# jeffreyhorn/network_flow_solver

Measured on AMD Instinct MI355X. Metric: pivots/sec + arcs-priced/sec (value = arcs-priced/sec; pivots_per_sec alongside) on netgen_8-style DIMACS, higher is better.
Workload: dtype int64; 1 GPU; netgen_8_08a(synthetic,x1): 256 nodes / 2048 arcs; pricing=full-scan Dantzig, step=one pivot (price + ratio test + tree/potential update), parallelism=1 GPU, sweeps=full (every arc priced every pivot)

## Files before the change

### __graft_entry__.py

```python

from __future__ import annotations

import os
import re
import subprocess
import sys
from pathlib import Path

ROOT = Path(__file__).resolve().parent
PKG = ROOT / "network_flow_solver_amd"
CSRC = PKG / "csrc"
LIB = PKG / "libmcf_hip.so"
CERT_HOST_LIB = PKG / "libmcf_certify_host.so"
REPAIR_HOST_LIB = PKG / "libmcf_repair_host.so"
FARKAS_HOST_LIB = PKG / "libmcf_farkas_host.so"
TOPOLOGY_HOST_LIB = PKG / "libmcf_topology_host.so"
RANGES_HOST_LIB = PKG / "libmcf_ranges_host.so"
FLOW_RANGES_HOST_LIB = PKG / "libmcf_flow_ranges_host.so"
DUAL_HOST_LIB = PKG / "libmcf_dual_host.so"
APPLY_PATHS_HOST_LIB = PKG / "libmcf_apply_paths_host.so"
SMALL_REDUCE_HOST_LIB = PKG / "libmcf_small_reduce_host.so"
SMALL_CYCLE_REGS_HOST_LIB = PKG / "libmcf_small_cycle_regs_host.so"
FORK_HOST_LIB = PKG / "libmcf_fork_host.so"

if str(ROOT) not in sys.path:
    sys.path.insert(0, str(ROOT))


def _hipcc() -> str:
    for cand in (os.environ.get("HIPCC"), "/opt/rocm/bin/hipcc", "hipcc"):
        if cand and (os.path.isabs(cand) and os.path.exists(cand) or not os.path.isabs(cand)):
            return cand
    return "hipcc"


def _needs_rebuild(target: Path, sources) -> bool:
    if not target.exists():
        return True
    t = target.stat().st_mtime
    return any(Path(s).stat().st_mtime > t for s in sources)


def build_hip(force: bool = False) -> Path:
    sources = [CSRC / "mcf_engine.hip", CSRC / "mcf_passes_dev.h", CSRC / "mcf_passes_host.h", CSRC / "mcf_core.h", CSRC / "mcf_host.h",
               ROOT / "include" / "mcf.h"]
    if force or _needs_rebuild(LIB, sources):
        cmd = [_hipcc(), "--offload-arch=gfx950", "-O3", "-std=c++17", "-fPIC", "-shared",
               "-o", str(LIB), str(CSRC / "mcf_engine.hip")]
        subprocess.run(cmd, check=True, cwd=str(CSRC))
    return LIB


def build_certify_host(force: bool = False) -> Path:
    src = CSRC / "mcf_certify_host.cpp"
    if force or _needs_rebuild(CERT_HOST_LIB, [src, CSRC / "mcf_core.h"]):
        subprocess.run(["g++", "-O2", "-std=c++17", "-fPIC", "-shared", "-o", str(CERT_HOST_LIB), str(src)], check=True, cwd=str(CSRC))
    return CERT_HOST_LIB


def build_repair_host(force: bool = False) -> Path:
    src = CSRC / "mcf_repair_host.cpp"
    if force or _needs_rebuild(REPAIR_HOST_LIB, [src, CSRC / "mcf_core.h", CSRC / "mcf_host.h"]):
        subprocess.run(["g++", "-O2", "-std=c++17", "-fPIC", "-shared", "-o", str(REPAIR_HOST_LIB), str(src)], check=True, cwd=str(CSRC))
    return REPAIR_HOST_LIB


def build_farkas_host(force: bool = False) -> Path:
    src = CSRC / "mcf_farkas_host.cpp"
    if force or _needs_rebuild(FARKAS_HOST_LIB, [src, CSRC / "mcf_core.h"]):
        subprocess.run(["g++", "-O2", "-std=c++17", "-fPIC", "-shared", "-o", str(FARKAS_HOST_LIB), str(src)], check=True, cwd=str(CSRC))
    return FARKAS_HOST_LIB


def build_topology_host(force: bool = False) -> Path:
    src = CSRC / "mcf_topology_host.cpp"
    if force or _needs_rebuild(TOPOLOGY_HOST_LIB, [src, CSRC / "mcf_core.h", CSRC / "mcf_host.h"]):
        subprocess.run(["g++", "-O2", "-std=c++17", "-fPIC", "-shared", "-o", str(TOPOLOGY_HOST_LIB), str(src)], check=True, cwd=str(CSRC))
    return TOPOLOGY_HOST_LIB


def build_ranges_host(force: bool = False) -> Path:
    src = CSRC / "mcf_ranges_host.cpp"
    if force or _needs_rebuild(RANGES_HOST_LIB, [src, CSRC / "mcf_core.h"]):
        subprocess.run(["g++", "-O2", "-std=c++17", "-fPIC", "-shared", "-o", str(RANGES_HOST_LIB), str(src)], check=True, cwd=str(CSRC))
    return RANGES_HOST_LIB


def build_flow_ranges_host(force: bool = False) -> Path:
    src = CSRC / "mcf_flow_ranges_host.cpp"
    if force or _needs_rebuild(FLOW_RANGES_HOST_LIB, [src, CSRC / "mcf_core.h"]):
        subprocess.run(["g++", "-O2", "-std=c++17", "-fPIC", "-shared", "-o", str(FLOW_RANGES_HOST_LIB), str(src)], check=True, cwd=str(CSRC))
    return FLOW_RANGES_HOST_LIB


def build_dual_host(force: bool = False) -> Path:
    src = CSRC / "mcf_dual_host.cpp"
    if force or _needs_rebuild(DUAL_HOST_LIB, [src, CSRC / "mcf_core.h", CSRC / "mcf_host.h", ROOT / "include" / "mcf.h"]):
        subprocess.run(["g++", "-O2", "-std=c++17", "-fPIC", "-shared", "-o", str(DUAL_HOST_LIB), str(src)], check=True, cwd=str(CSRC))
    return DUAL_HOST_LIB


def build_apply_paths_host(force: bool = False) -> Path:
    src = CSRC / "mcf_apply_paths_host.cpp"
    if force or _needs_rebuild(APPLY_PATHS_HOST_LIB, [src, CSRC / "mcf_core.h", CSRC / "mcf_host.h"]):
        subprocess.run(["g++", "-O2", "-std=c++17", "-fPIC", "-shared", "-o", str(APPLY_PATHS_HOST_LIB), str(src)], check=True, cwd=str(CSRC))
    return APPLY_PATHS_HOST_LIB


def build_small_reduce_host(force: bool = False) -> Path:
    src = CSRC / "mcf_small_reduce_host.cpp"
    if force or _needs_rebuild(SMALL_REDUCE_HOST_LIB, [src, CSRC / "mcf_core.h"]):
        subprocess.run(["g++", "-O2", "-std=c++17", "-fPIC", "-shared", "-o", str(SMALL_REDUCE_HOST_LIB), str(src)], check=True, cwd=str(CSRC))
    return SMALL_REDUCE_HOST_LIB


def build_small_cycle_regs_host(force: bool = False) -> Path:
    src = CSRC / "mcf_small_cycle_regs_host.cpp"
    if force or _needs_rebuild(SMALL_CYCLE_REGS_HOST_LIB, [src, CSRC / "mcf_core.h"]):
        subprocess.run(["g++", "-O2", "-std=c++17", "-fPIC", "-shared", "-o", str(SMALL_CYCLE_REGS_HOST_LIB), str(src)], check=True, cwd=str(CSRC))
    return SMALL_CYCLE_REGS_HOST_LIB


def build_fork_host(force: bool = False) -> Path:
    src = CSRC / "mcf_fork_host.cpp"
    if force or _needs_rebuild(FORK_HOST_LIB, [src, CSRC / "mcf_core.h"]):
        subprocess.run(["g++", "-O2", "-std=c++17", "-fPIC", "-shared", "-o", str(FORK_HOST_LIB), str(src)], check=True, cwd=str(CSRC))
    return FORK_HOST_LIB


def declared_symbols() -> list[str]:
    text = (ROOT / "include" / "mcf.h").read_text()
    text = re.sub(r"/\*.*?\*/", "", text, flags=re.S)
    names = re.findall(r"\b(mcf_[a-z0-9_]+)\s*\(", text)
    return sorted(set(n for n in names if n != "mcf_progress_cb"))


def build() -> None:
    build_hip()
    import oracle

    oracle.build()
    oracle.build_emul()
    build_certify_host()
    build_repair_host()
    build_farkas_host()
    build_topology_host()
    build_ranges_host()
    build_flow_ranges_host()
    build_dual_host()
    build_apply_paths_host()
    build_small_reduce_host()
    build_small_cycle_regs_host()
    build_fork_host()
    import ctypes

    lib = ctypes.CDLL(str(LIB))
    missing = [s for s in declared_symbols() if not hasattr(lib, s)]
    if missing:
        raise RuntimeError(f"libmcf_hip.so lacks symbols declared in include/mcf.h: {missing}")
    import network_flow_solver_amd


def smoke() -> None:
    import numpy as np

    build_hip()
    import oracle
    from network_flow_solver_amd import engine, generators

    if engine.device_count() <= 0:
        raise RuntimeError("smoke() needs a GPU: no HIP device visible")
    inst = generators.netgen_style(256, 2048, seed=7)
    ref = oracle.solve_soa(inst, "dantzig")
    for rule in (engine.RULE_DANTZIG, engine.RULE_DEVEX_BLOCK, engine.RULE_CANDIDATE_LIST):
        with engine.McfEngine(inst.n, inst.tail, inst.head, inst.cost, inst.cap, inst.supply, rule=rule,
                              device=0) as eng:
            eng.solve()
            res = eng.result()
        assert res.status == ref["status"] == "optimal", (res.status, ref["status"])
        assert res.objective == int(round(ref["objective"])), (res.objective, ref["objective"])
        bal = inst.supply.astype(np.int64).copy()
        np.subtract.at(bal, inst.tail, res.flow)
        np.add.at(bal, inst.head, res.flow)
        assert not bal.any()
        rc = inst.cost + res.potential[inst.tail] - res.potential[inst.head]
        assert (rc[(res.flow > 0) & (res.flow < inst.cap)] == 0).all()
        assert (rc[(res.flow == 0) & (inst.cap > 0)] >= 0).all() and (rc[(res.flow == inst.cap) & (inst.cap > 0)] <= 0).all()
        print(f"smoke ok: rule={rule} objective={res.objective} pivots={res.stats['pivots']} "
              f"(oracle {ref['iterations']} pivots)")


if __name__ == "__main__":
    build()
    if len(sys.argv) > 1 and sys.argv[1] == "smoke":
        smoke()
```

### network_flow_solver_amd/csrc/mcf_core.h

```cpp
#pragma once
#include <stdint.h>

#if defined(__HIPCC__)
#define MCF_HD __host__ __device__ __forceinline__
#else
#define MCF_HD inline
#endif

#define MCF_INF ((int64_t)1 << 60)

#if defined(__HIP_DEVICE_COMPILE__)
#define mcf_double_bits(x) ((int64_t)__double_as_longlong(x))
#else
static inline int64_t mcf_double_bits(double x) { int64_t k; __builtin_memcpy(&k, &x, 8); return k; }
#endif

#if defined(__HIP_DEVICE_COMPILE__)
#define MCF_TEAM_BARRIER() __syncthreads()
#define MCF_ATOMIC_MIN64(p, x) atomicMin(reinterpret_cast<long long*>(p), (long long)(x))
#define MCF_ATOMIC_MIN32(p, x) atomicMin(reinterpret_cast<int*>(p), (int)(x))
#define MCF_ATOMIC_MAX32(p, x) atomicMax(reinterpret_cast<int*>(p), (int)(x))
#define MCF_ATOMIC_ADD32(p, x) atomicAdd(reinterpret_cast<int*>(p), (int)(x))
#define MCF_ATOMIC_MAX64(p, x) atomicMax(reinterpret_cast<long long*>(p), (long long)(x))
#define MCF_ATOMIC_OR32(p, x) atomicOr(reinterpret_cast<int*>(p), (int)(x))
// ... 1107 lines not shown
        c->status = MCF_UNBOUNDED;
        c->unbounded_arc = e;
        return;
    }
    if (delta == 0) c->degenerate += 1;
    c->pivots += 1;
    c->cycle_arcs += n1 + n2 + 1;
    c->pv_e = e; c->pv_s = s; c->pv_n1 = n1; c->pv_n2 = n2; c->pv_delta = delta; c->pv_result = result;
    if (v.weight) {
        bool reset = false;
        if (result != 0) {
            if (c->swaps_since_reset >= MCF_DEVEX_RESET_SWAPS) { reset = true; c->swaps_since_reset = 0; }
            else c->swaps_since_reset += 1;
        }
        if (!reset && v.dx) {
            if (c->wlist_n >= MCF_WLIST_CAP) reset = true;
            else {
                const int32_t len = n1 + n2;
                v.weight[e] = (float)(len > 0 ? len : 1);
                v.dx->wlist[c->wlist_n] = e;
                c->wlist_n += 1;
            }
        }
        if (reset) { c->wreset = 1; c->block_index = 0; }
        c->tn_total += 1;
        if (delta == 0 || result == 0) c->tn_degenerate += 1;
        if (c->auto_tune && c->pivots - c->tn_last_adapt >= 50 && c->tn_total >= 10) {
            int32_t bg = c->block_granules;
            if (10 * c->tn_degenerate > 3 * c->tn_total) {
                const int32_t nb = bg * 3 / 2 > bg + 1 ? bg * 3 / 2 : bg + 1;
                bg = nb < c->max_granules ? nb : (bg > c->max_granules ? bg : c->max_granules);
            } else if (10 * c->tn_degenerate < c->tn_total) {
                const int32_t nb = bg * 3 / 4;
                bg = nb > 1 ? nb : 1;
            }
            if (bg != c->block_granules) {
                c->block_granules = bg;
                c->num_blocks = (MCF_GRANULES + bg - 1) / bg;
                c->block_size = v.m * bg / MCF_GRANULES;
                if (c->block_index >= c->num_blocks) c->block_index = 0;
            }
            c->tn_degenerate = 0; c->tn_total = 0; c->tn_last_adapt = c->pivots;
        }
    }
    if (result == 0) {
        c->bound_flips += 1;
        c->stage = 1;
        return;
    }

    mcf_pivot_swap(v, pp, cy, result, result == 1 ? k1 : k2, 0);
}

#define MCF_DUAL_FLOW_LIMIT ((int64_t)1 << 61)

MCF_HD int64_t mcf_dual_violation(int64_t cap, int64_t flow) {
    if (flow < 0) return -flow;
    return (cap < MCF_INF && flow > cap) ? flow - cap : 0;
}
MCF_HD int32_t mcf_dual_leave_state(int64_t flow) { return flow < 0 ? 1 : -1; }
MCF_HD bool mcf_dual_exports(bool up, int64_t flow) { return up == (flow >= 0); }
MCF_HD bool mcf_dual_candidate(int32_t state, int64_t cap, bool tail_in, bool head_in, bool exports) {
    if (state == 0 || cap == 0 || tail_in == head_in) return false;
    const bool first_in = state > 0 ? tail_in : head_in;
    return first_in == exports;
}
MCF_HD int32_t mcf_dual_closed_state(int32_t state, int64_t cap, int64_t rc) {
    return (state != 0 && cap == 0 && (int64_t)state * rc < 0) ? -state : state;
}
MCF_HD bool mcf_dual_in_subtree(int32_t pos, int32_t pos_q, int32_t size_q) { return pos >= pos_q && pos < pos_q + size_q; }

struct McfDualLeave { int64_t viol; int64_t node; int64_t maxabs; };
MCF_HD void mcf_acc_init(McfDualLeave* a) { a->viol = 0; a->node = -1; a->maxabs = 0; }
MCF_HD void mcf_dual_leave_add(McfDualLeave* a, int64_t viol, int64_t node, int64_t flow) {
    if (viol > 0 && (viol > a->viol || (viol == a->viol && (a->node < 0 || node < a->node)))) { a->viol = viol; a->node = node; }
    const int64_t mag = flow < 0 ? -flow : flow;
    if (mag > a->maxabs) a->maxabs = mag;
}
MCF_HD void mcf_acc_merge(McfDualLeave* a, const McfDualLeave& b) {
    if (b.node >= 0) mcf_dual_leave_add(a, b.viol, b.node, 0);
    if (b.maxabs > a->maxabs) a->maxabs = b.maxabs;
}
MCF_HD bool mcf_dual_too_large(const McfDualLeave& l) { return l.maxabs >= MCF_DUAL_FLOW_LIMIT || l.viol >= MCF_DUAL_FLOW_LIMIT; }
struct McfDualEnter { int64_t slack; int64_t arc; };
MCF_HD void mcf_acc_init(McfDualEnter* a) { a->slack = 0; a->arc = -1; }
MCF_HD void mcf_dual_enter_add(McfDualEnter* a, int64_t slack, int64_t packed_arc) {
    if (a->arc < 0 || slack < a->slack || (slack == a->slack && packed_arc < a->arc)) { a->slack = slack; a->arc = packed_arc; }
}
MCF_HD void mcf_acc_merge(McfDualEnter* a, const McfDualEnter& b) { if (b.arc >= 0) mcf_dual_enter_add(a, b.slack, b.arc); }

MCF_HD void mcf_pivot_begin_dual(const McfView& v, int64_t packed_arc, McfCycle* cy) {
    McfCtx* c = v.ctx;
    c->apply = 0;
    c->stage = 0;
    c->nchg = 0;
    if (c->wreset) { c->wreset = 0; c->wlist_n = 0; }
    if (c->pending_flip) {
        c->cur ^= 1;
        c->prev_lo = c->lo;
        c->prev_hi = c->hi;
        c->pending_flip = 0;
        if (c->rebuild) { c->arena ^= 1; c->rebuild = 0; }
    }
    if (packed_arc < 0) return;
    const int32_t e = (int32_t)(packed_arc & 0xffffffff);
    const McfArcW ae = v.arcw[e];
// ... 861 lines not shown
```

### network_flow_solver_amd/csrc/mcf_engine.hip

```cpp
#include <hip/hip_runtime.h>

#include <algorithm>
#include <cerrno>
#include <chrono>
#include <cstdio>
#include <cstdlib>
#include <cstring>
#include <mutex>
#include <new>
#include <string>
#include <vector>

#include "../../include/mcf.h"
#include "mcf_core.h"
#include "mcf_host.h"

namespace {

constexpr int kPriceThreads = 256;
constexpr int kPivotThreads = 1024;
constexpr int kReduceThreads = 256;
constexpr int kMidMaxNodes = 1536;
constexpr int kMidMaxArcsPerPivot = MCF_TUNER_MAX_ARCS + 1024;
constexpr int64_t kIncrementalMinArcs = (int64_t)1 << 22;
// ... 1287 lines not shown
template <int THREADS>
__device__ __forceinline__ void copy_words(void* dst, const void* src, uint32_t bytes) {
    const uint32_t n = bytes >> 2;
    const int32_t* s = static_cast<const int32_t*>(src);
    int32_t* d = static_cast<int32_t*>(dst);
    for (uint32_t i = threadIdx.x; i < n; i += THREADS) d[i] = s[i];
}

#ifdef MCF_STAMPS
#define STAMP(slot)                                                                       \
    do {                                                                                  \
        if (threadIdx.x == 0) {                                                           \
            const unsigned long long now_ = __builtin_amdgcn_s_memtime();                 \
            stamps_[slot] += now_ - last_;                                                \
            last_ = now_;                                                                 \
        }                                                                                 \
    } while (0)
#else
#define STAMP(slot) do {} while (0)
#endif
#ifdef MCF_STAMPS
#define MCF_LAST_WAVE_BEGIN() const unsigned long long lw0_ = __builtin_amdgcn_s_memtime()
#define MCF_LAST_WAVE_STAMP() do { last_wave_ += __builtin_amdgcn_s_memtime() - lw0_; } while (0)
#else
#define MCF_LAST_WAVE_BEGIN() do {} while (0)
#define MCF_LAST_WAVE_STAMP() do {} while (0)
#endif
#if defined(MCF_STAMPS) && defined(MCF_WAVE_STAMPS)
__shared__ unsigned long long mcf_wave_acc[16][6];
__shared__ unsigned long long mcf_wave_t0[16];
#define MCF_WAVE_T0() do { if ((threadIdx.x & 63) == 0) mcf_wave_t0[threadIdx.x >> 6] = __builtin_amdgcn_s_memtime(); } while (0)
#define MCF_WAVE_STAMP(slot)                                                                                                  \
    do { if ((threadIdx.x & 63) == 0) mcf_wave_acc[threadIdx.x >> 6][slot] += __builtin_amdgcn_s_memtime() - mcf_wave_t0[threadIdx.x >> 6]; } while (0)
#define MCF_WAVE_PROBE(word)                                                                                                  \
    do {                                                                                                                      \
        if (threadIdx.x < 64) {                                                                                               \
            const unsigned long long a_ = __builtin_amdgcn_s_memtime();                                                       \
            asm volatile("s_waitcnt lgkmcnt(0)" ::: "memory");                                                                \
            const unsigned long long b_ = __builtin_amdgcn_s_memtime();                                                       \
            asm volatile("s_waitcnt lgkmcnt(0)" ::: "memory");                                                                \
            const int32_t x_ = *reinterpret_cast<const volatile int32_t*>(word);                                              \
            asm volatile("s_waitcnt lgkmcnt(0)" ::"v"(x_) : "memory");                                                        \
            const unsigned long long c_ = __builtin_amdgcn_s_memtime();                                                       \
            asm volatile("s_waitcnt lgkmcnt(0)" ::: "memory");                                                                \
            if (threadIdx.x == 0) mcf_wave_acc[0][5] += (c_ - b_) - (b_ - a_);                                                \
        }                                                                                                                     \
    } while (0)
#else
#define MCF_WAVE_T0() do {} while (0)
#define MCF_WAVE_STAMP(slot) do {} while (0)
#define MCF_WAVE_PROBE(word) do {} while (0)
#endif

struct SmallCycleAcc {
    int32_t c1[16], c2[16];
};
constexpr bool small_search_join(int threads) { return threads != 256; }

template <bool LAST>
__device__ __forceinline__ void small_ratio_side(const int64_t* res, int32_t n, int64_t* d_out, int32_t* k_out) {
    const int32_t lane = (int32_t)(threadIdx.x & 63);
    int64_t d = MCF_INF;
    int32_t k = -1;
    const int64_t r0 = lane < n ? res[lane] : MCF_INF;
    bool wide = !mcf_ratio_narrow_ok(r0);
    for (int32_t i = 64 + lane; i < n; i += 64) wide |= !mcf_ratio_narrow_ok(res[i]);
    if (__ballot(wide) == 0) {
        for (int32_t base = 0; base < n; base += 64) {
            const int32_t i = base + lane;
            const uint32_t key = mcf_ratio_key32(base == 0 ? r0 : (i < n ? res[i] : MCF_INF));
            const uint32_t mn = mcf_wave_min_u32(key);
            const uint64_t mask = __ballot(i < n && key == mn);
            mcf_ratio_take<LAST>(mcf_ratio_unkey32(mn), mask, base, d, k);
        }
        *d_out = d; *k_out = k;
        return;
    }
    for (int32_t base = 0; base < n; base += 64) {
        const int32_t i = base + lane;
        const int64_t r = i < n ? res[i] : INT64_MAX;
        const int64_t mn = -mcf_wave_max64(-r);
        const uint64_t mask = __ballot(r == mn);
        mcf_ratio_take<LAST>(mn, mask, base, d, k);
    }
    *d_out = d; *k_out = k;
}

constexpr bool small_search_one_branch(int threads) { return threads == 256; }

constexpr bool small_ratio_together(int threads) { return threads == 256 || threads == 1024; }
constexpr bool small_record_once(int threads) { return threads == 256; }
typedef int small_i32x4 __attribute__((ext_vector_type(4)));

template <int THREADS>
__device__ __forceinline__ void small_cycle_parallel(const McfView& v, SmallCycleAcc& A, int64_t* scratch, McfCycle& cy) {
    constexpr bool kScalar = small_scalar_control(THREADS);
    constexpr bool kSearchJoin = small_search_join(THREADS);
    constexpr bool kSearchOneBranch = small_search_one_branch(THREADS);
    constexpr bool kRatioTogether = small_ratio_together(THREADS);
    constexpr bool kRecordOnce = small_record_once(THREADS);
    const McfCtx* c = v.ctx;
    const int32_t* pcur = c->cur ? v.posbuf[1] : v.posbuf[0];
    const int32_t du0 = cy.r0u.depth, dw0 = cy.r0w.depth;
    const int32_t pu = cy.p0u, pw = cy.p0w;
    const int32_t wave = (int32_t)threadIdx.x >> 6;
    const int32_t N = v.n_nodes;
    int64_t* const res1 = scratch;
    int64_t* const res2 = res1 + N;
    int32_t* const by_depth = reinterpret_cast<int32_t*>(res2 + N);
    int32_t n1w = 0, n2w = 0;
    const int32_t nx = kSearchJoin ? N : N - 1;
    for (int32_t x0 = 0; x0 < nx; x0 += THREADS) {
        const int32_t x = x0 + (int32_t)threadIdx.x;
        bool h1 = false, h2 = false;
        if (x < nx) {
            McfNode rec;
            if (kRecordOnce) {
                const small_i32x4 raw = *reinterpret_cast<const small_i32x4*>(&v.node[x]);
                rec.parent = raw.x; rec.pred = raw.y; rec.size = raw.z; rec.depth = raw.w;
            } else rec = v.node[x];
            const int32_t px = pcur[x];
            const bool au = (uint32_t)(pu - px) < (uint32_t)rec.size, aw = (uint32_t)(pw - px) < (uint32_t)rec.size;
            if (au && aw) { if (kSearchJoin) by_depth[rec.depth] = x; }
            else if (kSearchOneBranch) {
                if (au || aw) {
                    const McfArcW a = v.arcw[rec.pred >> 1];
                    const int32_t idx = (au ? du0 : dw0) - rec.depth;
                    (au ? v.path1 : v.path2)[idx] = x; (au ? v.rec1 : v.rec2)[idx] = rec; (au ? v.ppos1 : v.ppos2)[idx] = px;
                    const bool loses = ((rec.pred & 1) != 0) == au;
                    (au ? res1 : res2)[idx] = loses ? a.flow : (a.cap >= MCF_INF ? MCF_INF : a.cap - a.flow);
                    h1 = au; h2 = aw;
                }
            } else if (au) {
                const McfArcW a = v.arcw[rec.pred >> 1];
                const int32_t idx = du0 - rec.depth;
                v.path1[idx] = x; v.rec1[idx] = rec; v.ppos1[idx] = px;
                res1[idx] = (rec.pred & 1) ? a.flow : (a.cap >= MCF_INF ? MCF_INF : a.cap - a.flow);
                h1 = true;
            } else if (aw) {
                const McfArcW a = v.arcw[rec.pred >> 1];
                const int32_t idx = dw0 - rec.depth;
                v.path2[idx] = x; v.rec2[idx] = rec; v.ppos2[idx] = px;
                res2[idx] = (rec.pred & 1) ? (a.cap >= MCF_INF ? MCF_INF : a.cap - a.flow) : a.flow;
                h2 = true;
            }
        }
        n1w += (int32_t)__popcll(__ballot(h1));
        n2w += (int32_t)__popcll(__ballot(h2));
    }
    if ((threadIdx.x & 63) == 0) { A.c1[wave] = n1w; A.c2[wave] = n2w; }
    MCF_WAVE_STAMP(0);
    __syncthreads();
    int32_t n1 = 0, n2 = 0;
    int64_t d1, d2;
    int32_t k1, k2;
    {
        constexpr int kWaves = THREADS / 64;
        const int32_t lane = (int32_t)(threadIdx.x & 63);
        const int32_t c1 = lane < kWaves ? A.c1[lane] : 0, c2 = lane < kWaves ? A.c2[lane] : 0;
        const int32_t li = lane < N ? lane : N - 1;
        int64_t q1 = 0, q2 = 0;
        if (kRatioTogether) { q1 = res1[li]; q2 = res2[li]; }
#pragma unroll
        for (int q = 0; q < kWaves; ++q) { n1 += __builtin_amdgcn_readlane(c1, q); n2 += __builtin_amdgcn_readlane(c2, q); }
        bool both = false;
        if (kRatioTogether) {
            const int64_t r1 = lane < n1 ? q1 : MCF_INF, r2 = lane < n2 ? q2 : MCF_INF;
            const bool odd = !mcf_ratio_narrow_ok(r1) || !mcf_ratio_narrow_ok(r2);
            both = n1 <= 64 && n2 <= 64 && __ballot(odd) == 0;
            if (both) {
                const uint32_t key1 = mcf_ratio_key32(r1), key2 = mcf_ratio_key32(r2);
                uint32_t mn1, mn2;
                mcf_wave_min_u32_pair(key1, key2, mn1, mn2);
                const uint64_t mask1 = __ballot(lane < n1 && key1 == mn1), mask2 = __ballot(lane < n2 && key2 == mn2);
                d1 = MCF_INF; k1 = -1; d2 = MCF_INF; k2 = -1;
                if (n1 > 0) mcf_ratio_take<false>(mcf_ratio_unkey32(mn1), mask1, 0, d1, k1);
                if (n2 > 0) mcf_ratio_take<true>(mcf_ratio_unkey32(mn2), mask2, 0, d2, k2);
            }
        }
        if (!both) {
            small_ratio_side<false>(res1, n1, &d1, &k1);
            small_ratio_side<true>(res2, n2, &d2, &k2);
        }
    }
    cy.d1 = uni64<kScalar>(d1); cy.k1 = uni32<kScalar>(k1); cy.d2 = uni64<kScalar>(d2); cy.k2 = uni32<kScalar>(k2);
    cy.n1 = n1; cy.n2 = n2;
    MCF_WAVE_STAMP(1);
    if (kSearchJoin) {
        const int32_t jn = uni32<kScalar>(by_depth[du0 - n1]);
        const McfNode rj = uni_node<kScalar>(v.node[jn]);
        const int32_t pj = uni32<kScalar>(pcur[jn]);
        cy.u = jn; cy.w = jn; cy.ru = rj; cy.rw = rj;
        cy.pu = pj; cy.pw = pj; cy.su = pj; cy.sw = pj;
    }
}

enum { kSweepGeneric = 0, kSweepPlain = 1, kSweepDevex = 2 };

template <int MODE>
__device__ __forceinline__ void small_price_lds(const McfView& v, int32_t rule, bool devex, int32_t i, int64_t& key, int64_t& arc) {
    const int32_t st = v.state[i];
    const int32_t t = v.tail[i], h = v.head[i], o = v.orig[i];
    const int64_t cst = v.cost[i];
    float w = 1.0f;
    if (MODE == kSweepDevex || (MODE == kSweepGeneric && rule == MCF_RULE_DEVEX_BLOCK)) w = v.weight[i];
    const int64_t rc = cst + v.pi[t] - v.pi[h];
    const int64_t viol = st > 0 ? -rc : rc;
    if (st == 0 || viol <= 0) return;
    int64_t kk;
    int32_t id = o;
    if (MODE == kSweepPlain) kk = viol;
    else if (MODE == kSweepDevex) {
        kk = __double_as_longlong(((double)viol * (double)viol) / (double)w);
        id = mcf_devex_tie_id(o, st);
    } else {
        kk = mcf_dantzig_key(v, i, viol, st);
        if (rule == MCF_RULE_DEVEX_BLOCK) kk = __double_as_longlong(((double)viol * (double)viol) / (double)w);
        if (devex) id = mcf_devex_tie_id(o, st);
    }
    const int64_t pid = mcf_pack_arc(id, i);
    if (mcf_cand_better(kk, pid, key, arc)) { key = kk; arc = pid; }
}

__device__ __forceinline__ void half_wave_argmax(int64_t& key, int64_t& arc) {
    int64_t x = key;
    x = mcf_dpp_max_step<0xB1, 0xf>(x);
    x = mcf_dpp_max_step<0x4E, 0xf>(x);
    x = mcf_dpp_max_step<0x141, 0xf>(x);
    x = mcf_dpp_max_step<0x140, 0xf>(x);
    x = mcf_dpp_max_step<0x142, 0xa>(x);
    const int64_t m0 = readlane64(x, 31), m1 = readlane64(x, 63);
    const bool upper = (threadIdx.x & 32) != 0;
    const int64_t mx = upper ? m1 : m0;
    const uint64_t mask = __ballot(key == mx && key > 0);
    int64_t best[2] = {-1, -1};
#pragma unroll
    for (int hf = 0; hf < 2; ++hf) {
        uint64_t mk = hf ? (mask >> 32) << 32 : mask & 0xffffffffull;
        while (mk) {
            const int lane = __ffsll((unsigned long long)mk) - 1;
            const int64_t a = readlane64(arc, lane);
            if (best[hf] < 0 || a < best[hf]) best[hf] = a;
            mk &= mk - 1;
        }
    }
    const int64_t b = upper ? best[1] : best[0];
    key = b < 0 ? 0 : mx;
    arc = b;
}

constexpr bool small_desc_once(int threads, bool front) { return threads == 256 && !front; }
__device__ __forceinline__ uint32_t small_info(int32_t tail, int32_t head, int32_t q) { return (uint32_t)tail | ((uint32_t)head << 11) | ((uint32_t)q << 22); }
__device__ __forceinline__ McfCandX small_record(uint32_t info, int64_t viol, int32_t orig, int32_t e) {
    McfCandX x;
    x.state = (info >> 31) ? -1 : 1;
    x.rc = x.state > 0 ? -viol : viol;
    x.arc = mcf_pack_arc(orig, e);
    x.tail = (int32_t)(info & 0x7ff); x.head = (int32_t)((info >> 11) & 0x7ff); x.pad = 0;
    return x;
}
__device__ __forceinline__ void small_price_lds_narrow(const McfView& v, int32_t i, int32_t q, uint64_t& best, uint32_t& info) {
    const int32_t st = v.state[i];
    const int32_t t = v.tail[i], h = v.head[i], o = v.orig[i];
    const int32_t* pi32 = reinterpret_cast<const int32_t*>(v.pi);
    const int32_t rc = (int32_t)((uint32_t)v.cost[i] + (uint32_t)pi32[2 * t] - (uint32_t)pi32[2 * h]);
    const int32_t viol = st > 0 ? -rc : rc;
    const uint64_t p = ((uint64_t)(uint32_t)((st != 0 && viol > 0) ? viol : 0) << 32) | (uint32_t)~o;
    if (p > best) { best = p; info = small_info(t, h, q) | ((uint32_t)st & 0x80000000u); }
}
struct alignas(16) SmallWaveSlot {
    uint64_t key;
    int32_t e;
    uint32_t info;
};

#define MCF_SMALL_CTL_32(F)                                                                                                   \
    F(status) F(unbounded_arc) F(empty_blocks) F(num_blocks) F(block_granules) F(tn_total) F(tn_degenerate)                   \
    F(swaps_since_reset) F(wlist_n) F(wreset) F(minor_left) F(cur) F(pending_flip) F(prev_lo) F(prev_hi) F(apply) F(lo) F(hi) \
    F(nchg) F(stage) F(arena) F(rebuild)
#define MCF_SMALL_CTL_64(F)                                                                                                   \
    F(pivots) F(degenerate) F(bound_flips) F(arcs_priced) F(nodes_moved) F(subtree_nodes) F(cycle_arcs) F(block_size)         \
    F(block_index) F(tn_last_adapt) F(minor_pivots) F(major_sweeps)
#define MCF_SMALL_DESC_BEGIN_32(F) F(pv_e) F(pv_s) F(pv_first) F(pv_second) F(pv_t2n)
#define MCF_SMALL_DESC_BEGIN_64(F) F(pv_rc) F(pv_cap) F(pv_flow)
#define MCF_SMALL_DESC_DECIDE_32(F) F(pv_n1) F(pv_n2) F(pv_result)
#define MCF_SMALL_DESC_DECIDE_64(F) F(pv_delta)
#define MCF_SMALL_DESC_SWAP_32(F)                                                                                             \
    F(pv_k) F(pv_vin) F(pv_leave) F(pv_leave_state) F(pv_tail_in_t2) F(pv_vin_depth) F(pv_dd0) F(t2_old) F(t2_new) F(t2_size)  \
    F(nseg)
#define MCF_SMALL_DESC_SWAP_64(F) F(sigma)
template <bool SCALAR> __device__ __forceinline__ void small_ctx_uniform(McfCtx& x) {
#define MCF_F32(f) x.f = uni32<SCALAR>(x.f);
#define MCF_F64(f) x.f = uni64<SCALAR>(x.f);
    MCF_SMALL_CTL_32(MCF_F32) MCF_SMALL_CTL_64(MCF_F64)
    MCF_SMALL_DESC_BEGIN_32(MCF_F32) MCF_SMALL_DESC_BEGIN_64(MCF_F64)
    MCF_SMALL_DESC_DECIDE_32(MCF_F32) MCF_SMALL_DESC_DECIDE_64(MCF_F64)
    MCF_SMALL_DESC_SWAP_32(MCF_F32) MCF_SMALL_DESC_SWAP_64(MCF_F64)
    x.pv_t2node = uni32<SCALAR>(x.pv_t2node);
#undef MCF_F32
#undef MCF_F64
}
#define MCF_FST(f) c->f = x.f;
__device__ __forceinline__ void small_ctx_store(McfCtx* c, const McfCtx& x) {
    MCF_SMALL_CTL_32(MCF_FST) MCF_SMALL_CTL_64(MCF_FST)
// ... 200 lines not shown
    if (threadIdx.x == 0) { for (int i = 0; i < 24; ++i) mcf_stamp_acc[i] = 0; mcf_stamp_last = last_; }
#ifdef MCF_WAVE_STAMPS
    if (threadIdx.x < 16 * 6) (&mcf_wave_acc[0][0])[threadIdx.x] = 0;
#endif
#endif
    const SmallSizes sizes = small_sizes(g);
    McfView v = small_map_view<FRONT>(g, L, smem);
    small_copy_image<THREADS, true>(g, L, smem, v.weight != nullptr, sizes);
    __syncthreads();
    STAMP(0);

    McfCtx* const c = v.ctx;
    if (threadIdx.x == 0) arm_ctx(c, cap);
    __shared__ int32_t s_gran[MCF_NUM_BUCKETS][MCF_GRANULES + 1];
    const bool devex = !FRONT && rule == MCF_RULE_DEVEX_BLOCK && g.dx;
    small_load_granules<THREADS>(g, devex, s_gran);
    const bool listing = !FRONT && rule == MCF_RULE_CANDIDATE_LIST;
    __shared__ int64_t s_lk[MCF_NUM_BUCKETS], s_la[MCF_NUM_BUCKETS];
    if (listing && threadIdx.x < MCF_NUM_BUCKETS) { s_lk[threadIdx.x] = list[threadIdx.x].key; s_la[threadIdx.x] = list[threadIdx.x].arc; }
    __syncthreads();
    __shared__ int32_t s_gsum[MCF_GRANULES + 1];
    small_sum_granules(devex, s_gran, s_gsum);
    __syncthreads();
    constexpr bool kScalar = small_scalar_control(THREADS);
    const int64_t priced_all = uni32<kScalar>(s_gsum[MCF_GRANULES] - s_gsum[0]);

    constexpr int kPer = THREADS / MCF_NUM_BUCKETS;
    constexpr int kReg = small_reg_arcs(THREADS);
    static_assert(kPer == 32 || kPer % 64 == 0, "a head bucket's lanes are half a wave or whole waves");
    const int px = threadIdx.x / kPer, pl = threadIdx.x % kPer;
    const int sweep = FRONT ? (int)kSweepPlain
                            : (devex ? kSweepDevex : (rule != MCF_RULE_DEVEX_BLOCK && v.key_mode == MCF_KEY_PLAIN ? kSweepPlain : kSweepGeneric));
    int32_t r_tail[kReg], r_head[kReg], r_cost[kReg], r_orig[kReg];
    uint32_t r_info[kReg];
    int32_t r_n = 0;
    constexpr int kRegFew = small_reg_arcs_few(THREADS, FRONT);
    static_assert(kRegFew <= kReg, "the shorter unrolled sweep is a prefix of the longer");
    const bool even = FRONT && sweep == kSweepPlain && rule == MCF_RULE_DANTZIG;
    const int32_t r_step = even ? THREADS : kPer;
    const int32_t r_lo = even ? mcf_even_arc(s_gran[0][0], (int32_t)threadIdx.x, 0, THREADS) : s_gran[px][0] + pl;
    const int32_t r_hi = even ? s_gran[MCF_NUM_BUCKETS - 1][MCF_GRANULES] : s_gran[px][MCF_GRANULES];
    const bool r_few = even && uni32<kScalar>(mcf_even_reg_slots(s_gran[MCF_NUM_BUCKETS - 1][MCF_GRANULES] - s_gran[0][0], THREADS, kRegFew, kReg)) == kRegFew;
#pragma unroll
    for (int k = 0; k < kReg; ++k) {
        const int32_t i = r_lo + k * r_step;
        const bool on = sweep == kSweepPlain && i < r_hi;
        r_tail[k] = on ? v.tail[i] : 0; r_head[k] = on ? v.head[i] : 0; r_cost[k] = on ? v.cost[i] : 0; r_orig[k] = on ? v.orig[i] : 0;
        r_info[k] = small_info(r_tail[k], r_head[k], k);
        r_n += on ? 1 : 0;
    }
    const bool reg_plain = sweep == kSweepPlain;
    constexpr bool nar = FRONT;
    constexpr bool kDescOnce = small_desc_once(THREADS, FRONT);
    constexpr bool hand = FRONT;
    const int32_t* const pi32 = reinterpret_cast<const int32_t*>(v.pi);
    McfCtx cx = *c;
    small_ctx_uniform<kScalar>(cx);
    cx.max_pivots = uni64<kScalar>(cx.max_pivots); cx.minor_cap = uni32<kScalar>(cx.minor_cap); cx.auto_tune = uni32<kScalar>(cx.auto_tune);
    cx.devex_cyclic = uni32<kScalar>(cx.devex_cyclic); cx.max_granules = uni32<kScalar>(cx.max_granules);
    v.ctx = &cx;
    const int64_t adj2 = uni64<kScalar>(cx.pv_adj[2]), adj3 = uni64<kScalar>(cx.pv_adj[3]);
    int64_t* const scratch = reinterpret_cast<int64_t*>(smem + L.scratch);
    __shared__ McfCycle s_cy;
    __shared__ int s_ok;
    __shared__ SmallCycleAcc s_acc;
    __shared__ SmallWaveSlot s_slot[THREADS / 64];
    for (;;) {
        if (cx.status != MCF_RUNNING) break;
#if defined(MCF_STAMPS) && defined(MCF_WAVE_STAMPS)
        if ((cx.pivots & 15) == 0) { MCF_WAVE_PROBE(&s_acc.c1[0]); if (threadIdx.x == 64) mcf_wave_acc[1][5] += 1; }
#endif
        MCF_WAVE_T0();
        const bool minor = listing && cx.minor_left > 0;
        int32_t bg0, bg1;
        devex_block_granules(cx, devex, bg0, bg1);
        int64_t key = 0, arc = -1;
        McfCandX wx;
        wx.rc = 0; wx.arc = -1; wx.tail = 0; wx.head = 0; wx.state = 0; wx.pad = 0;
        uint64_t nbest = 0xffffffffull;
        uint32_t info = 0;
        if (!minor) {
            if (nar) {
                auto slots = [&](auto ns) {
                    constexpr int NS = decltype(ns)::value;
                    int32_t st[NS], pt[NS], ph[NS];
#pragma unroll
                    for (int k = 0; k < NS; ++k) {
                        st[k] = v.state[k < r_n ? r_lo + k * r_step : 0];
                        pt[k] = pi32[2 * r_tail[k]];
                        ph[k] = pi32[2 * r_head[k]];
                    }
#pragma unroll
                    for (int k = 0; k < NS; ++k) {
                        const int32_t rc = (int32_t)((uint32_t)r_cost[k] + (uint32_t)pt[k] - (uint32_t)ph[k]);
                        const int32_t s = k < r_n ? st[k] : 0;
                        const int32_t viol = s > 0 ? -rc : rc;
                        const uint64_t p = ((uint64_t)(uint32_t)((s != 0 && viol > 0) ? viol : 0) << 32) | (uint32_t)~r_orig[k];
                        if (p > nbest) { nbest = p; info = r_info[k] | ((uint32_t)s & 0x80000000u); }
                    }
                };
                if (r_few) slots(SmallSlots<kRegFew>{});
                else slots(SmallSlots<kReg>{});
                int32_t q = kReg;
                for (int32_t i = r_lo + kReg * r_step; i < r_hi; i += r_step, ++q) small_price_lds_narrow(v, i, q, nbest, info);
                if (nbest >> 32) { key = (int64_t)(nbest >> 32); arc = mcf_pack_arc((int32_t)~(uint32_t)nbest, r_lo + (int32_t)((info >> 22) & 0x1ff) * r_step); }
            } else if (reg_plain) {
                auto slots = [&](auto ns) {
                    constexpr int NS = decltype(ns)::value;
                    int32_t st[NS];
                    int64_t pt[NS], ph[NS];
#pragma unroll
                    for (int k = 0; k < NS; ++k) {
                        st[k] = v.state[k < r_n ? r_lo + k * r_step : 0];
                        pt[k] = v.pi[r_tail[k]];
                        ph[k] = v.pi[r_head[k]];
                    }
#pragma unroll
                    for (int k = 0; k < NS; ++k) {
                        const int64_t rc = (int64_t)r_cost[k] + pt[k] - ph[k];
                        const int32_t s = k < r_n ? st[k] : 0;
                        const int64_t viol = s > 0 ? -rc : rc;
                        const int64_t pid = mcf_pack_arc(r_orig[k], r_lo + k * r_step);
                        if (s != 0 && viol > 0 && mcf_cand_better(viol, pid, key, arc)) { key = viol; arc = pid; }
// ... 17 lines not shown
                    __shared__ int64_t s_wk[THREADS / 64], s_wa[THREADS / 64];
                    wave_argmax(key, arc);
                    if ((threadIdx.x & 63) == 0) { s_wk[threadIdx.x >> 6] = key; s_wa[threadIdx.x >> 6] = arc; }
                    __syncthreads();
                    if (threadIdx.x < MCF_NUM_BUCKETS) {
                        const int w = kWpb * threadIdx.x;
                        int64_t bk = s_wk[w], ba = s_wa[w];
                        for (int q = 1; q < kWpb; ++q)
                            if (mcf_cand_better(s_wk[w + q], s_wa[w + q], bk, ba)) { bk = s_wk[w + q]; ba = s_wa[w + q]; }
                        s_lk[threadIdx.x] = bk; s_la[threadIdx.x] = ba;
                    }
                } else {
                    half_wave_argmax(key, arc);
                    if (pl == 0) { s_lk[px] = key; s_la[px] = arc; }
                }
                __syncthreads();
            }
            const int32_t l = (int32_t)(threadIdx.x & 63);
            key = 0; arc = -1;
            if (l < MCF_NUM_BUCKETS) {
                arc = s_la[l];
                key = minor ? mcf_minor_key(v, arc) : s_lk[l];
                if (key <= 0) { key = 0; arc = -1; }
            }
            wave_argmax(key, arc);
        } else if constexpr (FRONT) {
            small_handover_publish(nbest, arc, info, s_slot);
            __syncthreads();
            small_handover_pick<THREADS>(s_slot, key, arc, wx);
        } else {
            block_argmax_all<THREADS>(key, arc);
        }
        STAMP(2);
        if (cx.pivots < cx.max_pivots)
            cx.arcs_priced += minor ? (int64_t)MCF_NUM_BUCKETS : (devex ? (int64_t)uni32<kScalar>(s_gsum[bg1] - s_gsum[bg0]) : priced_all);
        MCF_PSTAMP(12);
        McfCycle cy;
        bool go;
        if constexpr (hand) go = mcf_pivot_begin_t<true>(v, key, arc, rule, &wx, &cy);
        else go = mcf_pivot_begin_t<true>(v, key, arc, rule, nullptr, &cy);
        small_ctx_uniform<kScalar>(cx);
        MCF_PSTAMP(13);
        if (!go) {
            STAMP(3);
            __syncthreads();
            STAMP(5);
            continue;
        }
        small_cycle_ends<kScalar>(cy);
        const int32_t deep = cy.r0u.depth > cy.r0w.depth ? cy.r0u.depth : cy.r0w.depth;
        if (v.n_nodes <= kSmallCycleMaxNodes && deep > 3) {
            small_cycle_parallel<THREADS>(v, s_acc, scratch, cy);
            MCF_PSTAMP(15);
            mcf_pivot_decide(v, mcf_view_paths(v), cy);
        } else {
            if (threadIdx.x < 2) {
                const bool ok = pivot_climb_2lanes(v, &s_cy);
                if (threadIdx.x == 0) s_ok = ok ? 1 : 0;
            }
            __syncthreads();
            if (uni32<kScalar>(s_ok)) {
                cy = s_cy;
                uni_cycle<kScalar>(cy);
                mcf_pivot_decide(v, mcf_view_paths(v), cy);
            } else {
                cx.status = MCF_INTERNAL_ERROR;
            }
        }
        small_ctx_uniform<kScalar>(cx);
        if constexpr (!kDescOnce) { if (threadIdx.x == 0) small_desc_store(c, cx, adj2, adj3); }
        MCF_PSTAMP(16);
        STAMP(3);
        MCF_WAVE_STAMP(2);
        if ((int32_t)threadIdx.x >= THREADS - 64) {
            MCF_LAST_WAVE_BEGIN();
            mcf_pivot_finish_t<true>(v, mcf_view_paths(v), (int32_t)threadIdx.x - (THREADS - 64), 64);
            MCF_LAST_WAVE_STAMP();
            MCF_WAVE_STAMP(4);
        }
        STAMP(4);
        small_apply<THREADS, FRONT>(v, cx);
        MCF_WAVE_STAMP(3);
        __syncthreads();
        cx.apply = 0;
        STAMP(5);
    }
    if (threadIdx.x == 0) {
        small_ctx_store(c, cx);
        if constexpr (kDescOnce) small_desc_store_all(c, cx);
    }
    v.ctx = c;
    __syncthreads();
    __shared__ int s_any;
    small_budget_check<THREADS>(v, g, c, s_any);
    small_copy_image<THREADS, false>(g, L, smem, v.weight != nullptr, sizes);
    if (host_ctx) copy_words<THREADS>(host_ctx, smem + L.ctx, (uint32_t)sizeof(McfCtx));
    if (listing && threadIdx.x < MCF_NUM_BUCKETS) list[threadIdx.x] = McfCand{s_lk[threadIdx.x], s_la[threadIdx.x]};
#ifdef MCF_STAMPS
    STAMP(6);
    if (threadIdx.x == 0) {
        unsigned long long* out = reinterpret_cast<unsigned long long*>(g.rec1);
        for (int i = 0; i < 7; ++i) out[i] = stamps_[i];
        for (int i = 0; i < 24; ++i) g_pivot_stamps[i] += mcf_stamp_acc[i];
    }
    if (threadIdx.x == THREADS - 64) reinterpret_cast<unsigned long long*>(g.rec1)[7] = last_wave_;
#ifdef MCF_WAVE_STAMPS
    if (threadIdx.x < 16 * 6 && (int64_t)g.n_nodes * (int64_t)sizeof(McfNode) >= (8 + 16 * 6) * 8)
// ... 2080 lines not shown
```

Before: 640.7 million arcs/s.

## Use branch-free pivot decide and packed wave counts in small-graph kernel

Adds a branch-free, predicated version of mcf_pivot_decide for the 256-thread front path, so the leaving-arc and tree-update bookkeeping avoids divergent control flow. It also packs the per-wave cycle counts into int32 pairs that are read with a single vector load, adds asm barriers so the count and residual loads can be issued together, and turns on desc_once for the front path. A host-side exhaustive equivalence checker is added to compare the flat decide against the original. The risk is that the flat version always computes both sides and writes every ctx field, adding ALU work and stores.

```diff
diff --git a/__graft_entry__.py b/__graft_entry__.py
--- a/__graft_entry__.py
+++ b/__graft_entry__.py
@@ -22,6 +22,7 @@
 SMALL_REDUCE_HOST_LIB = PKG / "libmcf_small_reduce_host.so"
 SMALL_CYCLE_REGS_HOST_LIB = PKG / "libmcf_small_cycle_regs_host.so"
 FORK_HOST_LIB = PKG / "libmcf_fork_host.so"
+DECIDE_FLAT_HOST_LIB = PKG / "libmcf_decide_flat_host.so"
 
 if str(ROOT) not in sys.path:
     sys.path.insert(0, str(ROOT))
@@ -126,6 +127,13 @@
     if force or _needs_rebuild(FORK_HOST_LIB, [src, CSRC / "mcf_core.h"]):
         subprocess.run(["g++", "-O2", "-std=c++17", "-fPIC", "-shared", "-o", str(FORK_HOST_LIB), str(src)], check=True, cwd=str(CSRC))
     return FORK_HOST_LIB
+
+
+def build_decide_flat_host(force: bool = False) -> Path:
+    src = CSRC / "mcf_decide_flat_host.cpp"
+    if force or _needs_rebuild(DECIDE_FLAT_HOST_LIB, [src, CSRC / "mcf_core.h"]):
+        subprocess.run(["g++", "-O2", "-std=c++17", "-fPIC", "-shared", "-o", str(DECIDE_FLAT_HOST_LIB), str(src)], check=True, cwd=str(CSRC))
+    return DECIDE_FLAT_HOST_LIB
 
 
 def declared_symbols() -> list[str]:
@@ -152,6 +160,7 @@
     build_small_reduce_host()
     build_small_cycle_regs_host()
     build_fork_host()
+    build_decide_flat_host()
     import ctypes
 
     lib = ctypes.CDLL(str(LIB))
diff --git a/network_flow_solver_amd/csrc/mcf_core.h b/network_flow_solver_amd/csrc/mcf_core.h
--- a/network_flow_solver_amd/csrc/mcf_core.h
+++ b/network_flow_solver_amd/csrc/mcf_core.h
@@ -1183,6 +1183,73 @@
     mcf_pivot_swap(v, pp, cy, result, result == 1 ? k1 : k2, 0);
 }
 
+MCF_HD void mcf_pivot_decide_flat(const McfView& v, const McfPaths& pp, const McfCycle& cy) {
+    McfCtx* c = v.ctx;
+    const int32_t e = c->pv_e, s = c->pv_s, first = c->pv_first, second = c->pv_second;
+    const int64_t d1 = cy.d1, d2 = cy.d2, rc = c->pv_rc;
+    const int32_t n1 = cy.n1, n2 = cy.n2;
+    const int64_t de = c->pv_cap;
+    const bool take2 = d2 <= de && d2 <= d1;
+    const bool take0 = !take2 && de <= d1;
+    const bool side1 = !take2 && !take0;
+    const int32_t result = take2 ? 2 : (take0 ? 0 : 1);
+    const int64_t delta = take2 ? d2 : (take0 ? de : d1);
+    const int32_t kq = side1 ? cy.k1 : cy.k2;
+    const int32_t k = (take0 || kq < 0) ? 0 : kq;
+    const McfNode rq = (side1 ? pp.rec1 : pp.rec2)[k];
+    const int32_t a0 = (side1 ? pp.ppos1 : pp.ppos2)[k];
+    const bool live = delta < MCF_INF;
+    const bool flip = live && take0;
+    const bool swap = live && !take0;
+
+    c->status = live ? c->status : (int32_t)MCF_UNBOUNDED;
+    c->unbounded_arc = live ? c->unbounded_arc : e;
+    c->degenerate += (live && delta == 0) ? 1 : 0;
+    c->pivots += live ? 1 : 0;
+    c->cycle_arcs += live ? n1 + n2 + 1 : 0;
+    c->pv_n1 = live ? n1 : c->pv_n1;
+    c->pv_n2 = live ? n2 : c->pv_n2;
+    c->pv_delta = live ? delta : c->pv_delta;
+    c->pv_result = live ? result : c->pv_result;
+    c->bound_flips += flip ? 1 : 0;
+
+    const bool tail_in_t2 = side1 == (s > 0);
+    const int32_t S = rq.size;
+    const int32_t du0 = cy.r0u.depth, dw0 = cy.r0w.depth, zu0 = cy.r0u.size, zw0 = cy.r0w.size;
+    const int32_t vin_depth = side1 ? dw0 : du0, vin_size = side1 ? zw0 : zu0;
+    const int32_t pvin = side1 ? cy.p0w : cy.p0u;
+    const int32_t tA = pvin + 1, tB = pvin + vin_size;
+    const int32_t costA = tA <= a0 ? a0 - tA : tA - (a0 + S);
+    const int32_t costB = tB <= a0 ? a0 - tB : tB - (a0 + S);
+    const int32_t t = costA <= costB ? tA : tB;
+    const int32_t lo = t < a0 ? t : a0, hi = t > a0 + S ? t : a0 + S;
+    c->pv_k = swap ? k : c->pv_k;
+    c->pv_vin = swap ? (side1 ? second : first) : c->pv_vin;
+    c->pv_leave = swap ? (rq.pred >> 1) : c->pv_leave;
+    c->pv_leave_state = swap ? ((((rq.pred & 1) != 0) == side1) ? 1 : -1) : c->pv_leave_state;
+    c->pv_tail_in_t2 = swap ? (tail_in_t2 ? 1 : 0) : c->pv_tail_in_t2;
+    c->sigma = swap ? (tail_in_t2 ? -rc : rc) : c->sigma;
+    c->pv_vin_depth = swap ? vin_depth : c->pv_vin_depth;
+    c->pv_dd0 = swap ? vin_depth + 1 - (side1 ? du0 : dw0) : c->pv_dd0;
+    c->t2_old = swap ? a0 : c->t2_old;
+    c->t2_new = swap ? (t <= a0 ? t : t - S) : c->t2_new;
+    c->t2_size = swap ? S : c->t2_size;
+    c->lo = swap ? lo : c->lo;
+    c->hi = swap ? hi : c->hi;
+    c->nseg = swap ? 2 * k + 1 : c->nseg;
+    c->nchg = swap ? (side1 ? n1 : n2) - k - 1 : c->nchg;
+    c->apply = swap ? 1 : c->apply;
+    c->pending_flip = swap ? 1 : c->pending_flip;
+    c->subtree_nodes += swap ? S : 0;
+    c->nodes_moved += swap ? hi - lo : 0;
+    c->stage = swap ? 2 : (flip ? 1 : c->stage);
+    const bool one = swap && S == 1, move = one && !side1;
+    c->pv_t2n = one ? 1 : c->pv_t2n;
+    c->pv_t2node = one ? (side1 ? first : second) : c->pv_t2node;
+    c->pv_adj[0] = move ? c->pv_adj[2] : c->pv_adj[0];
+    c->pv_adj[1] = move ? c->pv_adj[3] : c->pv_adj[1];
+}
+
 #define MCF_DUAL_FLOW_LIMIT ((int64_t)1 << 61)
 
 MCF_HD int64_t mcf_dual_violation(int64_t cap, int64_t flow) {
diff --git a/network_flow_solver_amd/csrc/mcf_decide_flat_driver.cpp b/network_flow_solver_amd/csrc/mcf_decide_flat_driver.cpp
--- /dev/null
+++ b/network_flow_solver_amd/csrc/mcf_decide_flat_driver.cpp
@@ -0,0 +1,12 @@
+#include <cstdint>
+#include <cstdio>
+
+extern "C" int mcf_decide_flat_sweep_host(int64_t* counts);
+
+int main() {
+    int64_t counts[24];
+    const int rc = mcf_decide_flat_sweep_host(counts);
+    for (int i = 0; i < 24; ++i) std::printf(i ? " %lld" : "%lld", (long long)counts[i]);
+    std::printf("\n");
+    return rc == 0 ? 0 : 1;
+}
diff --git a/network_flow_solver_amd/csrc/mcf_decide_flat_host.cpp b/network_flow_solver_amd/csrc/mcf_decide_flat_host.cpp
--- /dev/null
+++ b/network_flow_solver_amd/csrc/mcf_decide_flat_host.cpp
@@ -0,0 +1,140 @@
+#include <cstdint>
+#include <cstring>
+
+#include "mcf_core.h"
+
+namespace {
+
+const int64_t kBig = ((int64_t)1 << 32);
+const int64_t kResiduals[6] = {0, 1, 5, kBig - 2, kBig + 5, MCF_INF};
+const int32_t kSide = 4;
+const int32_t kA0 = 20;
+
+struct Place { int32_t pos, size_base, size_per_s; };
+const Place kPlaces[7] = {
+    {10, 1, 0},
+    {10, 5, 0},
+    {30, 5, 0},
+    {10, 40, 0},
+    {10, 10, 1},
+    {10, 19, 1},
+    {5, 17, 1},
+};
+
+struct Case {
+    int64_t d1, d2, cap;
+    int32_t s, parity, S, kpos, minus, place;
+};
+
+void junk_ctx(McfCtx* c, uint32_t seed) {
+    uint32_t words[sizeof(McfCtx) / 4];
+    for (size_t i = 0; i < sizeof(McfCtx) / 4; ++i) {
+        seed = seed * 1664525u + 1013904223u;
+        words[i] = 1u + ((seed >> 8) & 0xfffffu);
+    }
+    std::memcpy(c, words, sizeof(McfCtx));
+}
+
+int run_case(const Case& q, McfCtx* ref_out, int32_t* k_leave) {
+    McfCtx start;
+    junk_ctx(&start, 12345u + (uint32_t)q.place * 7919u + (uint32_t)q.kpos);
+    start.status = MCF_RUNNING;
+    start.apply = 0; start.stage = 0; start.nchg = 0;
+    start.pv_e = 77; start.pv_s = q.s; start.pv_first = 41; start.pv_second = 42;
+    start.pv_rc = q.s > 0 ? -9 : 9;
+    start.pv_cap = q.cap;
+
+    const int leaves = (q.d2 <= q.cap && q.d2 <= q.d1) ? 2 : (q.cap <= q.d1 ? 0 : 1);
+    McfCycle cy;
+    std::memset(&cy, 0, sizeof(cy));
+    cy.d1 = q.d1; cy.d2 = q.d2;
+    const int32_t kk = q.kpos == 2 ? kSide - 1 : q.kpos;
+    cy.k1 = q.d1 < MCF_INF ? kk : -1;
+    cy.k2 = q.d2 < MCF_INF ? kk : -1;
+    if (q.minus) { if (leaves != 1) cy.k1 = -1; if (leaves != 2) cy.k2 = -1; }
+    cy.n1 = kSide; cy.n2 = kSide;
+    const Place& pu = kPlaces[q.place];
+    const Place& pw = kPlaces[(q.place + 3) % 7];
+    cy.p0u = pu.pos; cy.r0u.size = pu.size_base + pu.size_per_s * q.S; cy.r0u.depth = 6; cy.r0u.parent = 3; cy.r0u.pred = 12;
+    cy.p0w = pw.pos; cy.r0w.size = pw.size_base + pw.size_per_s * q.S; cy.r0w.depth = 9; cy.r0w.parent = 4; cy.r0w.pred = 15;
+    *k_leave = leaves == 1 ? cy.k1 : (leaves == 2 ? cy.k2 : -1);
+
+    McfNode rec1[kSide], rec2[kSide];
+    int32_t ppos1[kSide], ppos2[kSide], path1[kSide], path2[kSide];
+    for (int32_t j = 0; j < kSide; ++j) {
+        const bool q1 = j == cy.k1, q2 = j == cy.k2;
+        rec1[j].parent = 100 + j; rec1[j].pred = ((7 + j) << 1) | q.parity; rec1[j].size = q1 ? q.S : q.S + 5 + j; rec1[j].depth = 5 - j;
+        rec2[j].parent = 200 + j; rec2[j].pred = ((57 + j) << 1) | q.parity; rec2[j].size = q2 ? q.S : q.S + 6 + j; rec2[j].depth = 8 - j;
+        ppos1[j] = q1 ? kA0 : 200 + 10 * j;
+        ppos2[j] = q2 ? kA0 : 300 + 10 * j;
+        path1[j] = 500 + j; path2[j] = 600 + j;
+    }
+    McfPaths pp;
+    std::memset(&pp, 0, sizeof(pp));
+    pp.path1 = path1; pp.path2 = path2; pp.rec1 = rec1; pp.rec2 = rec2; pp.ppos1 = ppos1; pp.ppos2 = ppos2;
+    pp.slot1 = ppos1; pp.slot2 = ppos2;
+
+    McfCtx a = start, b = start;
+    McfView v;
+    std::memset(&v, 0, sizeof(v));
+    v.n_nodes = 64;
+    v.ctx = &a;
+    mcf_pivot_decide(v, pp, cy);
+    v.ctx = &b;
+    mcf_pivot_decide_flat(v, pp, cy);
+    *ref_out = a;
+    if (std::memcmp(&a, &b, sizeof(McfCtx)) == 0) return 0;
+    const unsigned char *pa = reinterpret_cast<const unsigned char*>(&a), *pb = reinterpret_cast<const unsigned char*>(&b);
+    for (size_t i = 0; i < sizeof(McfCtx); ++i)
+        if (pa[i] != pb[i]) return 1 + (int)i;
+    return 1;
+}
+
+}
+
+extern "C" {
+
+enum { MCF_DECIDE_FLAT_COUNTS = 24 };
+
+int mcf_decide_flat_sweep_host(int64_t* counts) {
+    if (!counts) return -1;
+    for (int i = 0; i < MCF_DECIDE_FLAT_COUNTS; ++i) counts[i] = 0;
+    counts[22] = -1; counts[23] = -1;
+    Case q;
+    for (int i1 = 0; i1 < 6; ++i1) for (int i2 = 0; i2 < 6; ++i2) for (int ic = 0; ic < 6; ++ic)
+    for (int s = -1; s <= 1; s += 2) for (int parity = 0; parity < 2; ++parity) for (int S = 1; S <= 3; S += 2)
+    for (int kpos = 0; kpos < 3; ++kpos) for (int minus = 0; minus < 2; ++minus) for (int place = 0; place < 7; ++place) {
+        q.d1 = kResiduals[i1]; q.d2 = kResiduals[i2]; q.cap = kResiduals[ic];
+        q.s = s; q.parity = parity; q.S = S; q.kpos = kpos; q.minus = minus; q.place = place;
+        McfCtx r;
+        int32_t k = -1;
+        const int bad = run_case(q, &r, &k);
+        if (bad) { if (counts[1] == 0) { counts[22] = counts[0]; counts[23] = bad - 1; } counts[1] += 1; }
+        counts[0] += 1;
+        if (r.status == MCF_UNBOUNDED) { counts[2] += 1; continue; }
+        if (r.pv_delta == 0) counts[6] += 1;
+        if (r.stage == 1) { counts[3] += 1; continue; }
+        if (r.stage != 2) return -2;
+        counts[r.pv_result == 1 ? 4 : 5] += 1;
+        const Place& pl = kPlaces[r.pv_result == 1 ? (place + 3) % 7 : place];
+        const int32_t tA = pl.pos + 1, tB = pl.pos + pl.size_base + pl.size_per_s * S;
+        const int32_t costA = tA <= kA0 ? kA0 - tA : tA - (kA0 + S), costB = tB <= kA0 ? kA0 - tB : tB - (kA0 + S);
+        const int32_t t = costA <= costB ? tA : tB;
+        if (r.t2_old != kA0 || r.t2_size != S || r.pv_k != k) return -3;
+        if (r.t2_new != (t <= kA0 ? t : t - S) || r.lo != (t < kA0 ? t : kA0) || r.hi != (t > kA0 + S ? t : kA0 + S)) return -4;
+        if (tA != tB) counts[t == tA ? 7 : 8] += 1;
+        if (tA != tB && costA == costB) counts[9] += 1;
+        counts[t <= kA0 ? 10 : (t == kA0 + S ? 11 : 12)] += 1;
+        if (S == 1) counts[r.pv_result == 1 ? 13 : 14] += 1;
+        if (S == 3) counts[21] += 1;
+        if (minus) counts[15] += 1;
+        counts[k == 0 ? 16 : (k == 1 ? 17 : 18)] += 1;
+        counts[19] |= 1 << parity;
+        counts[20] |= s > 0 ? 1 : 2;
+    }
+    return counts[1] == 0 ? 0 : 1;
+}
+
+int32_t mcf_decide_flat_ctx_bytes_host(void) { return (int32_t)sizeof(McfCtx); }
+
+}
diff --git a/network_flow_solver_amd/csrc/mcf_engine.hip b/network_flow_solver_amd/csrc/mcf_engine.hip
--- a/network_flow_solver_amd/csrc/mcf_engine.hip
+++ b/network_flow_solver_amd/csrc/mcf_engine.hip
@@ -1363,8 +1363,8 @@
 #define MCF_WAVE_PROBE(word) do {} while (0)
 #endif
 
-struct SmallCycleAcc {
-    int32_t c1[16], c2[16];
+struct alignas(8) SmallCycleAcc {
+    int32_t c[16][2];
 };
 constexpr bool small_search_join(int threads) { return threads != 256; }
 
@@ -1402,6 +1402,8 @@
 constexpr bool small_ratio_together(int threads) { return threads == 256 || threads == 1024; }
 constexpr bool small_record_once(int threads) { return threads == 256; }
 typedef int small_i32x4 __attribute__((ext_vector_type(4)));
+constexpr bool small_ratio_one_trip(int threads) { return threads == 256; }
+typedef int small_i32x2 __attribute__((ext_vector_type(2)));
 
 template <int THREADS>
 __device__ __forceinline__ void small_cycle_parallel(const McfView& v, SmallCycleAcc& A, int64_t* scratch, McfCycle& cy) {
@@ -1410,6 +1412,7 @@
     constexpr bool kSearchOneBranch = small_search_one_branch(THREADS);
     constexpr bool kRatioTogether = small_ratio_together(THREADS);
     constexpr bool kRecordOnce = small_record_once(THREADS);
+    constexpr bool kRatioOneTrip = kRatioTogether && small_ratio_one_trip(THREADS);
     const McfCtx* c = v.ctx;
     const int32_t* pcur = c->cur ? v.posbuf[1] : v.posbuf[0];
     const int32_t du0 = cy.r0u.depth, dw0 = cy.r0w.depth;
@@ -1459,7 +1462,7 @@
         n1w += (int32_t)__popcll(__ballot(h1));
         n2w += (int32_t)__popcll(__ballot(h2));
     }
-    if ((threadIdx.x & 63) == 0) { A.c1[wave] = n1w; A.c2[wave] = n2w; }
+    if ((threadIdx.x & 63) == 0) { A.c[wave][0] = n1w; A.c[wave][1] = n2w; }
     MCF_WAVE_STAMP(0);
     __syncthreads();
     int32_t n1 = 0, n2 = 0;
@@ -1468,19 +1471,27 @@
     {
         constexpr int kWaves = THREADS / 64;
         const int32_t lane = (int32_t)(threadIdx.x & 63);
-        const int32_t c1 = lane < kWaves ? A.c1[lane] : 0, c2 = lane < kWaves ? A.c2[lane] : 0;
+        int32_t c1, c2;
+        if (kRatioOneTrip) {
+            const small_i32x2 cc = *reinterpret_cast<const small_i32x2*>(&A.c[lane < kWaves ? lane : kWaves - 1][0]);
+            c1 = cc.x; c2 = cc.y;
+        } else {
+            c1 = lane < kWaves ? A.c[lane][0] : 0; c2 = lane < kWaves ? A.c[lane][1] : 0;
+        }
         const int32_t li = lane < N ? lane : N - 1;
         int64_t q1 = 0, q2 = 0;
         if (kRatioTogether) { q1 = res1[li]; q2 = res2[li]; }
+        if (kRatioOneTrip) asm volatile("" ::"v"(c1), "v"(c2), "v"(q1), "v"(q2));
 #pragma unroll
         for (int q = 0; q < kWaves; ++q) { n1 += __builtin_amdgcn_readlane(c1, q); n2 += __builtin_amdgcn_readlane(c2, q); }
         bool both = false;
         if (kRatioTogether) {
             const int64_t r1 = lane < n1 ? q1 : MCF_INF, r2 = lane < n2 ? q2 : MCF_INF;
             const bool odd = !mcf_ratio_narrow_ok(r1) || !mcf_ratio_narrow_ok(r2);
+            uint32_t key1 = mcf_ratio_key32(r1), key2 = mcf_ratio_key32(r2);
+            if (kRatioOneTrip) asm volatile("" : "+v"(key1), "+v"(key2));
             both = n1 <= 64 && n2 <= 64 && __ballot(odd) == 0;
             if (both) {
-                const uint32_t key1 = mcf_ratio_key32(r1), key2 = mcf_ratio_key32(r2);
                 uint32_t mn1, mn2;
                 mcf_wave_min_u32_pair(key1, key2, mn1, mn2);
                 const uint64_t mask1 = __ballot(lane < n1 && key1 == mn1), mask2 = __ballot(lane < n2 && key2 == mn2);
@@ -1560,7 +1571,8 @@
     arc = b;
 }
 
-constexpr bool small_desc_once(int threads, bool front) { return threads == 256 && !front; }
+constexpr bool small_desc_once(int threads, bool front) { return threads == 256; }
+constexpr bool small_decide_flat(int threads, bool front) { return threads == 256 && front; }
 __device__ __forceinline__ uint32_t small_info(int32_t tail, int32_t head, int32_t q) { return (uint32_t)tail | ((uint32_t)head << 11) | ((uint32_t)q << 22); }
 __device__ __forceinline__ McfCandX small_record(uint32_t info, int64_t viol, int32_t orig, int32_t e) {
     McfCandX x;
@@ -1867,6 +1879,7 @@
     const bool reg_plain = sweep == kSweepPlain;
     constexpr bool nar = FRONT;
     constexpr bool kDescOnce = small_desc_once(THREADS, FRONT);
+    constexpr bool kDecideFlat = small_decide_flat(THREADS, FRONT);
     constexpr bool hand = FRONT;
     const int32_t* const pi32 = reinterpret_cast<const int32_t*>(v.pi);
     McfCtx cx = *c;
@@ -1883,7 +1896,7 @@
     for (;;) {
         if (cx.status != MCF_RUNNING) break;
 #if defined(MCF_STAMPS) && defined(MCF_WAVE_STAMPS)
-        if ((cx.pivots & 15) == 0) { MCF_WAVE_PROBE(&s_acc.c1[0]); if (threadIdx.x == 64) mcf_wave_acc[1][5] += 1; }
+        if ((cx.pivots & 15) == 0) { MCF_WAVE_PROBE(&s_acc.c[0][0]); if (threadIdx.x == 64) mcf_wave_acc[1][5] += 1; }
 #endif
         MCF_WAVE_T0();
         const bool minor = listing && cx.minor_left > 0;
@@ -2007,7 +2020,8 @@
         if (v.n_nodes <= kSmallCycleMaxNodes && deep > 3) {
             small_cycle_parallel<THREADS>(v, s_acc, scratch, cy);
             MCF_PSTAMP(15);
-            mcf_pivot_decide(v, mcf_view_paths(v), cy);
+            if constexpr (kDecideFlat) mcf_pivot_decide_flat(v, mcf_view_paths(v), cy);
+            else mcf_pivot_decide(v, mcf_view_paths(v), cy);
         } else {
             if (threadIdx.x < 2) {
                 const bool ok = pivot_climb_2lanes(v, &s_cy);
```

Result: faster. 668.2 million arcs/s (median of 6 runs) (+4.3%).
